# nils-werner/pymf

Measured on AMD Instinct MI355X. Metric: factorize_iters_per_sec, higher is better.
Workload: dtype f32

## Files before the change

pymf_amd/csrc/build.py:

```python
import hashlib
import os
import subprocess
import sys

HERE = os.path.dirname(os.path.abspath(__file__))
OUT = os.path.join(HERE, "libpymf_hip.so")
STAMP = OUT + ".srchash"
DEPS = sorted(f for f in os.listdir(HERE) if f.endswith((".h", ".hip"))) + \
       [os.path.join("..", "..", "include", "pymf_hip.h")]
FLAGS = ["--offload-arch=gfx950", "-O3", "-std=c++17", "-shared", "-fPIC", "-Wno-unused-result",
         "-mllvm", "-amdgpu-mfma-vgpr-form=1"]


def source_hash():
    h = hashlib.sha256()
    h.update(" ".join(FLAGS).encode())
    for d in DEPS:
        p = os.path.join(HERE, d)
        h.update(b"\0" + d.encode() + b"\0")
        with open(p, "rb") as f:
            h.update(f.read())
    return h.hexdigest()


def built_hash():
    try:
        with open(STAMP) as f:
            return f.read().strip()
    except OSError:
        return None


def up_to_date():
    return os.path.exists(OUT) and built_hash() == source_hash()


UNITS = ["pmf_nnls_quad_tu.hip", "pmf_api.hip", "pmf_nnls_tu.hip", "pmf_fused_tu.hip"]


def build(force=False, verbose=True):
    if not force and up_to_date():
        return OUT
    hipcc = os.environ.get("HIPCC", "/opt/rocm/bin/hipcc")
    want = source_hash()
    if os.path.exists(STAMP):
        os.remove(STAMP)
    cflags = [f for f in FLAGS if f != "-shared"]
    objs, procs = [], []
    for u in UNITS:
        obj = os.path.join(HERE, u.replace(".hip", ".o"))
        cmd = [hipcc] + cflags + ["-c", os.path.join(HERE, u), "-o", obj]
        if verbose:
            print(" ".join(cmd), flush=True)
        procs.append((cmd, subprocess.Popen(cmd, cwd=HERE)))
        objs.append(obj)
    for cmd, pr in procs:
        if pr.wait() != 0:
            for _, other in procs:
                if other.poll() is None:
                    other.kill()
            raise subprocess.CalledProcessError(pr.returncode, cmd)
    link = [hipcc, "--offload-arch=gfx950", "-shared", "-fPIC"] + objs + ["-o", OUT, "-lrccl"]
    if verbose:
        print(" ".join(link), flush=True)
    subprocess.check_call(link, cwd=HERE)
    for o in objs:
        os.remove(o)
    if source_hash() != want:
        raise RuntimeError("sources changed while libpymf_hip.so was being built: build again")
    with open(STAMP, "w") as f:
        f.write(want + "\n")
    return OUT


if __name__ == "__main__":
    build(force="--force" in sys.argv)
```

pymf_amd/csrc/pmf_fused.h:

```cpp
#pragma once
#include "pmf_dev.h"
#include <hip/hip_ext.h>
#include "../../include/pymf_hip.h"
#include "pmf_fused_api.h"

#define PMF_GLDS16(gsrc, ldst)                                                            \
  __builtin_amdgcn_global_load_lds((const __attribute__((address_space(1))) void*)(gsrc), \
                                   (__attribute__((address_space(3))) void*)(ldst), 16, 0, 0)

#ifdef PMF_STAMPS
#define PMF_STAMP(var)                                                           \
  do {                                                                           \
    __builtin_amdgcn_sched_barrier(0);                                           \
    asm volatile("s_memtime %0\n\ts_waitcnt lgkmcnt(0)" : "=s"(var)::"memory"); \
    __builtin_amdgcn_sched_barrier(0);                                           \
  } while (0)
#else
#define PMF_STAMP(var) do { } while (0)
#endif


__device__ __forceinline__ void slab_store16(f32x4* p, f32x4 v) { *p = v; }
__device__ __forceinline__ void wrow_store(float* p, float v) { *p = v; }

template <int N>
__device__ __forceinline__ void wait_vmcnt() {
  static_assert(N >= 0 && N < 64, "vmcnt range");
  asm volatile("s_waitcnt vmcnt(%0)" ::"n"(N) : "memory");
}

template <int NT, int NPANEL, int SPLIT = 1>
constexpr size_t fused_smem_bytes() {
  return (size_t)64 * (SPLIT * NPANEL * 16 * NT + 16 * NT + 4 * 16 * NPANEL + 4 * 16) * sizeof(float) +
         (SPLIT == 2 ? (size_t)4 * NT * 1024 : 0);
}

__device__ __forceinline__ int vtile_xor(int row) { return (row ^ ((row & 4) << 1)) & 15; }
__device__ __forceinline__ int vtile_off(int row, int chunk) { return row * 64 + ((chunk ^ vtile_xor(row)) << 2); }
__device__ __forceinline__ f32x4 vtile_read4(const float* base, int row, int chunk) {
  return *reinterpret_cast<const f32x4*>(base + vtile_off(row, chunk));
}

template <int NT, int NPANEL, int MODE, int SPLIT = 1>
__global__ __launch_bounds__(256, 1) void k_nmf_fused(const float* __restrict__ V,
                                                       float* __restrict__ W,
                                                       const float* __restrict__ H,
                                                       const float* __restrict__ G, int blk_per,
                                                       int blk_extra, float lamb,
                                                       float* __restrict__ slab,
                                                       const FusedCtl ctl, int ngp
#ifdef PMF_STAMPS
                                                       , unsigned long long* __restrict__ dbg
#endif
                                                       ) {
  constexpr int KP = 16 * NT;
  static_assert(SPLIT == 1 || (SPLIT == 2 && MODE != FUSED_SNMF), "SPLIT: 1, or 2 for the NMF/BNMF epilogues");
  constexpr int NPT = NPANEL * SPLIT;
  constexpr int NP = 64 * NPT;
  constexpr int NTP = 4 * NPANEL;
  constexpr bool SPREAD = (NPANEL == 4);
  constexpr bool SNMF = (MODE == FUSED_SNMF);
  if (ctl.stop != nullptr && *ctl.stop != 0) return;
#ifdef PMF_STAMPS
  unsigned long long tk0 = 0, tk1 = 0, tk2 = 0, tk3 = 0;
  const unsigned long long rt0 = wall_clock64();
  PMF_STAMP(tk0);
#endif
  extern __shared__ __attribute__((aligned(16))) float smem[];
  float* sH = smem;
  float* sG = sH + NPT * KP * 64;
  float* sVall = sG + KP * 64;
  float* sWall = sVall + 4 * NPANEL * 16 * 64;
  const int tid = threadIdx.x, lane = tid & 63;
  const int wv = __builtin_amdgcn_readfirstlane(tid >> 6);
  const int i = lane & 15, kq = lane >> 4;
  float* sV = sVall + wv * (NPANEL * 1024);
  float* sW = sWall + wv * 1024;
  f32x4* sX = reinterpret_cast<f32x4*>(sWall + 4 * 1024);
  const int half = SPLIT == 2 ? (wv & 1) : 0;
  const int hp = half * NPANEL;

  const int gw = SPLIT == 2 ? blockIdx.x * 2 + (wv >> 1) : blockIdx.x * 4 + wv;
  const int b0 = gw * blk_per + (gw < blk_extra ? gw : blk_extra);
  const int nb = blk_per + (gw < blk_extra ? 1 : 0);
  const int nb_wg = blk_per + (blk_extra > 0 ? 1 : 0);
  constexpr bool interleave = NT == 1;
  const int nw_all = (int)gridDim.x * (SPLIT == 2 ? 2 : 4);
  const int bfirst = interleave ? gw : b0;
  const int bstep = interleave ? nw_all : 1;

  unsigned voff[4], woff[4];
#pragma unroll
  for (int q = 0; q < 4; ++q) {
    const int row = 4 * q + (lane >> 4);
    const int c = (lane & 15) ^ vtile_xor(row);
    voff[q] = (unsigned)(row * NP * 4 + 16 * c);
    woff[q] = (unsigned)(row * KP * 4 + 16 * (4 * c < KP ? c : 0));
  }
  const char* Vb = reinterpret_cast<const char*>(V);
  const char* Wb = reinterpret_cast<const char*>(W);
  auto issue_v = [&](int blk, int p, int q) {
    PMF_GLDS16(Vb + ((size_t)blk * (16 * NP * 4) + (hp + p) * 256) + voff[q], sV + p * 1024 + q * 256);
  };
  auto issue_w = [&](int blk, int q) {
    PMF_GLDS16(Wb + (size_t)blk * (16 * KP * 4) + woff[q], sW + q * 256);
  };

  f32x4 P[NT][NTP];
  f32x4 S[NT][NT];
#pragma unroll
  for (int mt = 0; mt < NT; ++mt) {
#pragma unroll
    for (int nt = 0; nt < NTP; ++nt) P[mt][nt] = f32x4{0.f, 0.f, 0.f, 0.f};
#pragma unroll
    for (int nt = 0; nt < NT; ++nt) S[mt][nt] = f32x4{0.f, 0.f, 0.f, 0.f};
  }

  constexpr int HP = SPLIT * NT;
  constexpr int GP = SNMF ? 0 : NT;
  constexpr int WP = SNMF ? 0 : 4;
  {
    const int drow = lane >> 4, dchunk = lane & 15;
#pragma unroll
    for (int st = 0; st < NPANEL; ++st) {
#pragma unroll
      for (int hh = 0; hh < SPLIT; ++hh)
#pragma unroll
        for (int u = 0; u < NT; ++u) {
          const int p = hh * NPANEL + st, rg = 4 * u + wv;
          const int row = 4 * rg + drow;
          const int bas = NT * (row & 15) + (row >> 4);
          const float* src = H + (size_t)bas * NP + 64 * p + 4 * (dchunk ^ (row & 15));
          PMF_GLDS16(src, sH + p * (KP * 64) + rg * 256);
        }
      if (nb > 0 && (st < NPANEL - 1 || !SPREAD)) {
#pragma unroll
        for (int q = 0; q < 4; ++q) issue_v(bfirst, st, q);
      }
      if (st == 0 && !SNMF && nb > 0) {
#pragma unroll
        for (int q = 0; q < 4; ++q) issue_w(bfirst, q);
      }
    }
#pragma unroll
    for (int u = 0; u < (SNMF ? 0 : NT); ++u) {
      const int rg = 4 * u + wv;
      const int row = 4 * rg + drow;
      const int bas = NT * (row & 15) + (row >> 4);
      int c = dchunk ^ (row & 15);
      if (4 * c >= KP) c = 0;
      if (ngp == 0) {
        PMF_GLDS16(G + bas * KP + 4 * c, sG + rg * 256);
      } else {
        f32x4 g = {0.f, 0.f, 0.f, 0.f};
        for (int w = 0; w < ngp; ++w)
          g += *reinterpret_cast<const f32x4*>(G + (size_t)w * KP * KP + bas * KP + 4 * c);
        *reinterpret_cast<f32x4*>(sG + rg * 256 + drow * 64 + dchunk * 4) = g;
      }
    }
  }
  if (ctl.stop != nullptr && ctl.conv_iter >= 0) {
    double t0 = ctl.tt[0], t1 = ctl.tt[1];
    for (int q = 1; q < ctl.ntt; ++q) { t0 += ctl.tt[2 * q]; t1 += ctl.tt[2 * q + 1]; }
    const double e2 = ctl.vnorm2 - 2.0 * t0 + t1;
    int st = 0;
    if (!(e2 > 1e-3 * ctl.vnorm2)) {
      st = 2;
    } else {
      const double f = sqrt(e2);
      if (blockIdx.x == 0 && tid == 0) ctl.ferr[ctl.conv_iter] = f;
      if (ctl.conv_iter > 1 && fabs(f - ctl.ferr[ctl.conv_iter - 1]) / ctl.nsamp < ctl.eps) st = 1;
    }
    if (st != 0) {
      if (blockIdx.x == 0 && tid == 0) { ctl.stop[1] = ctl.conv_iter; ctl.stop[0] = st; }
      return;
    }
  }
  auto wg_barrier = [&]() {
    asm volatile("s_waitcnt lgkmcnt(0)" ::: "memory");
    __builtin_amdgcn_s_barrier();
    asm volatile("" ::: "memory");
  };
  auto first_stage = [&](int st) {
    if (st >= NPANEL - 1) wait_vmcnt<0>();
    else if (SPREAD) {
      if (st == 0) wait_vmcnt<WP + 2 * (HP + 4) + HP + GP>();
      else if (st == 1) wait_vmcnt<(HP + 4) + HP + GP + 3>();
      else wait_vmcnt<HP + GP + 4>();
    } else {
      if (st == 0) wait_vmcnt<WP + (NPANEL - 1) * (HP + 4) + GP>();
      else if (st == 1) wait_vmcnt<(NPANEL > 2 ? (NPANEL - 2) * (HP + 4) : 0) + GP>();
      else if (st == 2) wait_vmcnt<(NPANEL > 3 ? (NPANEL - 3) * (HP + 4) : 0) + GP>();
      else if (st == 3) wait_vmcnt<(NPANEL > 4 ? (NPANEL - 4) * (HP + 4) : 0) + GP>();
      else wait_vmcnt<0>();
    }
    wg_barrier();
  };
  if (nb == 0) {
    wait_vmcnt<0>();
#pragma unroll
    for (int st = 0; st < NPANEL; ++st) wg_barrier();
  }

  f32x4 fa[2];
  f32x4 fb[2][NT];
  f32x4 bf[2];
  f32x4 wp[NT];
#pragma unroll
  for (int nt = 0; nt < NT; ++nt) wp[nt] = f32x4{0.f, 0.f, 0.f, 0.f};

  constexpr int NSN = 4 * NPANEL;
  constexpr int NSA = SNMF ? NSN : NSN + NT;

#ifdef PMF_STAMPS
  PMF_STAMP(tk1);
  unsigned long long ts0 = 0, ts1 = 0, ts2 = 0, ts3 = 0, ts4 = 0, ts5 = 0;
  unsigned long long acc_wait = 0, acc_a = 0, acc_dma = 0, acc_epi = 0, acc_b = 0;
#endif
  for (int b = 0; b < (SPLIT == 2 ? nb_wg : nb); ++b) {
    if (SPLIT == 2) {
      wg_barrier();
      if (b >= nb) { wg_barrier(); continue; }
    }
    const int blk = bfirst + b * bstep;
    const bool more = (b + 1 < nb);
    PMF_STAMP(ts0);

    f32x4 num[NT], den[NT];
#pragma unroll
    for (int nt = 0; nt < NT; ++nt) {
      num[nt] = f32x4{0.f, 0.f, 0.f, 0.f};
      den[nt] = f32x4{0.f, 0.f, 0.f, 0.f};
    }
    auto load_step = [&](int s, int buf) {
      if (s < NSN) {
        const int p = s >> 2, chunk = 4 * (s & 3) + kq;
        fa[buf] = vtile_read4(sV + p * 1024, i, chunk);
#pragma unroll
        for (int nt = 0; nt < NT; ++nt) fb[buf][nt] = lds_read4(sH + (hp + p) * (KP * 64), 16 * nt + i, chunk);
      } else {
        const int chunk = 4 * (s - NSN) + kq;
        fa[buf] = vtile_read4(sW, i, chunk);
#pragma unroll
        for (int nt = 0; nt < NT; ++nt) fb[buf][nt] = lds_read4(sG, 16 * nt + i, chunk);
      }
    };
    auto wait_panel = [&](int p) {
      if (SPREAD) {
        if (p == 0) wait_vmcnt<8>();
        else if (p == 1) wait_vmcnt<7>();
        else if (p == 2) wait_vmcnt<4>();
        else wait_vmcnt<0>();
      } else {
        if (p == 0) wait_vmcnt<4 * (NPANEL - 1)>();
        else if (p == 1) wait_vmcnt<(NPANEL > 1 ? 4 * (NPANEL - 2) : 0)>();
        else if (p == 2) wait_vmcnt<(NPANEL > 2 ? 4 * (NPANEL - 3) : 0)>();
        else wait_vmcnt<0>();
      }
    };

    const bool first = (b == 0);
    if (first) first_stage(0);
    else wait_panel(0);
    PMF_STAMP(ts1);
    load_step(0, 0);
#pragma unroll
    for (int s = 0; s < NSA; ++s) {
      if (s + 1 < NSA) {
        if (s + 1 < NSN && ((s + 1) & 3) == 0) {
          if (first) first_stage((s + 1) >> 2);
          else wait_panel((s + 1) >> 2);
        }
        load_step(s + 1, (s + 1) & 1);
      }
      const int buf = s & 1;
      if (s < NSN) {
#pragma unroll
        for (int e = 0; e < 4; ++e)
#pragma unroll
          for (int nt = 0; nt < NT; ++nt) num[nt] = mfma16(fa[buf][e], fb[buf][nt][e], num[nt]);
      } else {
#pragma unroll
        for (int e = 0; e < 4; ++e)
#pragma unroll
          for (int nt = 0; nt < NT; ++nt) den[nt] = mfma16(fa[buf][e], fb[buf][nt][e], den[nt]);
      }
      if (SPREAD && s < 4) issue_v(blk, NPANEL - 1, s);
      if (s + 1 < NSA) {
#pragma unroll
        for (int g = 0; g < NT + 1; ++g) {
          __builtin_amdgcn_sched_group_barrier(0x008, NT >= 4 ? 2 : 1, 0);
          __builtin_amdgcn_sched_group_barrier(0x100, 1, 0);
        }
      }
      __builtin_amdgcn_sched_group_barrier(0x008, 4 * NT, 0);
      __builtin_amdgcn_sched_barrier(0);
    }
    if (SPLIT == 2) {
#pragma unroll
      for (int nt = 0; nt < NT; ++nt) sX[(wv * NT + nt) * 64 + lane] = num[nt];
      wg_barrier();
#pragma unroll
      for (int nt = 0; nt < NT; ++nt) num[nt] += sX[((wv ^ 1) * NT + nt) * 64 + lane];
    }
    PMF_STAMP(ts2);
    float wold[NT][4];
    if (!SNMF) {
#pragma unroll
      for (int nt = 0; nt < NT; ++nt)
#pragma unroll
        for (int j = 0; j < 4; ++j) {
          const int row = 4 * kq + j, col = NT * i + nt;
          wold[nt][j] = sW[vtile_off(row, col >> 2) + (col & 3)];
        }
      asm volatile("s_waitcnt lgkmcnt(0)" ::: "memory");
      if (more) {
#pragma unroll
        for (int q = 0; q < 4; ++q) issue_w(blk + bstep, q);
      }
    }
    PMF_STAMP(ts3);

    f32x4 wn[NT];
    float* wdst = W + (size_t)blk * (16 * KP) + (4 * kq) * KP + NT * i;
    if (MODE != FUSED_SNMF) {
      float tnum[NT][4], dd[NT][4], rr[NT][4], qq[NT][4];
      constexpr int NSM = 4 * (NT * (NT + 1) / 2);
      auto s_mfmas = [&](int lo, int hi) {
        if (SPLIT == 1 || half == 0) {
          int q = 0;
#pragma unroll
          for (int j = 0; j < 4; ++j)
#pragma unroll
            for (int nt = 0; nt < NT; ++nt)
#pragma unroll
              for (int mt = 0; mt <= nt; ++mt) {
                if (q >= lo && q < hi) S[mt][nt] = mfma16(wp[mt][j], wp[nt][j], S[mt][nt]);
                ++q;
              }
        }
      };
#pragma unroll
      for (int nt = 0; nt < NT; ++nt)
#pragma unroll
        for (int j = 0; j < 4; ++j) {
          const float w0 = wold[nt][j];
          if (MODE == FUSED_BNMF) {
            tnum[nt][j] = num[nt][j] + (3.0f * lamb) * (w0 * w0);
            dd[nt][j] = ((den[nt][j] + (2.0f * lamb) * (w0 * w0 * w0)) + lamb * w0) + PMF_EPS_DEN;
          } else if (MODE == FUSED_RNMF) {
            const float x = num[nt][j];
            tnum[nt][j] = fabsf(x) - x;
            dd[nt][j] = 2.0f * den[nt][j];
          } else {
            tnum[nt][j] = w0 * num[nt][j];
            dd[nt][j] = den[nt][j] + PMF_EPS_DEN;
          }
        }
      s_mfmas(0, NSM / 5);
      __builtin_amdgcn_sched_barrier(0);
#pragma unroll
      for (int nt = 0; nt < NT; ++nt)
#pragma unroll
        for (int j = 0; j < 4; ++j) rr[nt][j] = __builtin_amdgcn_rcpf(dd[nt][j]);
      s_mfmas(NSM / 5, 2 * NSM / 5);
      __builtin_amdgcn_sched_barrier(0);
#pragma unroll
      for (int nt = 0; nt < NT; ++nt)
#pragma unroll
        for (int j = 0; j < 4; ++j) qq[nt][j] = tnum[nt][j] * rr[nt][j];
      s_mfmas(2 * NSM / 5, 3 * NSM / 5);
      __builtin_amdgcn_sched_barrier(0);
#pragma unroll
      for (int nt = 0; nt < NT; ++nt)
#pragma unroll
        for (int j = 0; j < 4; ++j) tnum[nt][j] = fmaf(-dd[nt][j], qq[nt][j], tnum[nt][j]);
      s_mfmas(3 * NSM / 5, 4 * NSM / 5);
      __builtin_amdgcn_sched_barrier(0);
#pragma unroll
      for (int nt = 0; nt < NT; ++nt)
#pragma unroll
        for (int j = 0; j < 4; ++j) {
          float w = fmaf(tnum[nt][j], rr[nt][j], qq[nt][j]);
          if (MODE == FUSED_BNMF) w = wold[nt][j] * w;
          if (MODE == FUSED_RNMF) w = dd[nt][j] != 0.f ? wold[nt][j] * w : 0.f;
          wn[nt][j] = w;
          if (SPLIT == 1 || half == 0) wrow_store(&wdst[j * KP + nt], w);
        }
      s_mfmas(4 * NSM / 5, NSM);
      __builtin_amdgcn_sched_barrier(0);
    } else {
#pragma unroll
      for (int nt = 0; nt < NT; ++nt)
#pragma unroll
        for (int j = 0; j < 4; ++j) {
          const float w = num[nt][j];
          wn[nt][j] = w;
          wrow_store(&wdst[j * KP + nt], w);
#pragma unroll
          for (int mt = 0; mt <= nt; ++mt) S[mt][nt] = mfma16(wp[mt][j], wp[nt][j], S[mt][nt]);
        }
    }
#pragma unroll
    for (int nt = 0; nt < NT; ++nt) wp[nt] = wn[nt];

    PMF_STAMP(ts4);
    auto load_bf = [&](int s, int buf) {
      const int p = s >> 2, row = 4 * kq + (s & 3);
      bf[buf] = vtile_read4(sV + p * 1024, row, i);
    };
    load_bf(0, 0);
#pragma unroll
    for (int s = 0; s < NSN; ++s) {
      if (s + 1 < NSN) load_bf(s + 1, (s + 1) & 1);
      const int p = s >> 2, j = s & 3, buf = s & 1;
#pragma unroll
      for (int mt = 0; mt < NT; ++mt)
#pragma unroll
        for (int nt = 0; nt < 4; ++nt)
          P[mt][4 * p + nt] = mfma16(wn[mt][j], bf[buf][nt], P[mt][4 * p + nt]);
      if (SPREAD) {
        if (p >= 1 && more) issue_v(blk + bstep, p - 1, j);
      }
      if (s + 1 < NSN) {
        __builtin_amdgcn_sched_group_barrier(0x008, NT >= 2 ? 2 : 1, 0);
        __builtin_amdgcn_sched_group_barrier(0x100, 1, 0);
      }
      __builtin_amdgcn_sched_barrier(0);
      if (!SPREAD && j == 3) {
        asm volatile("s_waitcnt lgkmcnt(0)" ::: "memory");
        if (more) {
#pragma unroll
          for (int q = 0; q < 4; ++q) issue_v(blk + bstep, p, q);
        }
      }
    }
    if (SPREAD) asm volatile("s_waitcnt lgkmcnt(0)" ::: "memory");
#ifdef PMF_STAMPS
    PMF_STAMP(ts5);
    acc_wait += ts1 - ts0; acc_a += ts2 - ts1; acc_dma += ts3 - ts2; acc_epi += ts4 - ts3; acc_b += ts5 - ts4;
#endif
  }
#ifdef PMF_STAMPS
  PMF_STAMP(tk2);
#endif
  if (SPLIT == 1 || half == 0) {
#pragma unroll
    for (int j = 0; j < 4; ++j)
#pragma unroll
      for (int nt = 0; nt < NT; ++nt)
#pragma unroll
        for (int mt = 0; mt <= nt; ++mt) S[mt][nt] = mfma16(wp[mt][j], wp[nt][j], S[mt][nt]);
  }

  constexpr int NTU = NT * NTP + NT * (NT + 1) / 2;
  __syncthreads();
  f32x4* ex = reinterpret_cast<f32x4*>(smem);
  static_assert((size_t)2 * NTU * 64 * 16 <= fused_smem_bytes<NT, NPANEL, SPLIT>(), "exchange fits");
  auto put = [&](int region) {
    f32x4* dst = ex + (size_t)region * NTU * 64 + lane;
#pragma unroll
    for (int mt = 0; mt < NT; ++mt) {
#pragma unroll
      for (int nt = 0; nt < NTP; ++nt) dst[(mt * NTP + nt) * 64] = P[mt][nt];
#pragma unroll
      for (int nt = mt; nt < NT; ++nt)
        dst[(NT * NTP + mt * NT - (mt * (mt - 1)) / 2 + (nt - mt)) * 64] = S[mt][nt];
    }
  };
  auto add = [&](int region) {
    const f32x4* src = ex + (size_t)region * NTU * 64 + lane;
#pragma unroll
    for (int mt = 0; mt < NT; ++mt) {
#pragma unroll
      for (int nt = 0; nt < NTP; ++nt) P[mt][nt] += src[(mt * NTP + nt) * 64];
#pragma unroll
      for (int nt = mt; nt < NT; ++nt)
        S[mt][nt] += src[(NT * NTP + mt * NT - (mt * (mt - 1)) / 2 + (nt - mt)) * 64];
    }
  };
  if (wv >= 2) put(wv - 2);
  __syncthreads();
  if (wv < 2) add(wv);
  __syncthreads();
  if (wv < 2) put(wv);
  __syncthreads();
  if (SPLIT == 1) {
    f32x4* out = reinterpret_cast<f32x4*>(slab) + (size_t)blockIdx.x * NTU * 64 + lane;
    for (int t = wv; t < NTU; t += 4)
      slab_store16(&out[t * 64], ex[t * 64 + lane] + ex[(size_t)NTU * 64 + t * 64 + lane]);
  } else {
    constexpr int NTPT = 4 * NPT, NTUT = NT * NTPT + NT * (NT + 1) / 2;
    f32x4* out = reinterpret_cast<f32x4*>(slab) + (size_t)blockIdx.x * NTUT * 64 + lane;
    for (int t = wv; t < 2 * NT * NTP; t += 4) {
      const int h = t / (NT * NTP), q = t % (NT * NTP), mt = q / NTP, nt = q % NTP;
      slab_store16(&out[(mt * NTPT + h * NTP + nt) * 64], ex[(size_t)h * NTU * 64 + q * 64 + lane]);
    }
    for (int t = wv; t < NT * (NT + 1) / 2; t += 4)
      slab_store16(&out[(NT * NTPT + t) * 64], ex[(NT * NTP + t) * 64 + lane]);
  }
#ifdef PMF_STAMPS
  PMF_STAMP(tk3);
  if (dbg && lane == 0) {
    unsigned long long* d = dbg + ((size_t)blockIdx.x * 4 + wv) * 12;
    d[0] = acc_wait; d[1] = acc_a; d[2] = acc_dma; d[3] = acc_epi; d[4] = acc_b; d[5] = (unsigned long long)nb;
    d[6] = tk1 - tk0; d[7] = tk3 - tk2;
    d[8] = rt0; d[9] = wall_clock64(); d[10] = tk3 - tk0; d[11] = tk2 - tk1;
  }
#endif
}

#ifndef PMF_FUSED_KERNEL_ONLY
static inline bool fused_shape_ok(int NT, int np) {
  const int npanel = np / 64;
  if (np % 64 != 0 || npanel < 1) return false;
  const int max_panels = NT == 1 ? 6 : NT == 2 ? 5 : NT == 4 ? 4 : 0;
  return npanel <= max_panels;
}

static inline bool fused_shape_split(int NT, int np) {
  if (NT == 2) return np == 384 || np == 512;
  if (NT == 1) return np == 512;
  return false;
}

static inline int fused_grid_for(int NT, int np, int64_t mp, bool allow_split = true) {
  const bool split = allow_split && !fused_shape_ok(NT, np) && fused_shape_split(NT, np);
  if (!fused_shape_ok(NT, np) && !split) return 0;
  int dev = 0, cus = 256;
  hipDeviceProp_t prop;
  if (hipGetDevice(&dev) == hipSuccess && hipGetDeviceProperties(&prop, dev) == hipSuccess)
    cus = prop.multiProcessorCount;
  const int64_t nblk = mp / 16;
  int64_t wgs = split ? (nblk + 1) / 2 : (nblk + 3) / 4;
  if (wgs > cus) wgs = cus;
  return (int)wgs;
}

static inline const char* fused_kernel_name(int NT, int np, int mode = FUSED_NMF) {
  static char buf[64];
  const bool split = !fused_shape_ok(NT, np) && fused_shape_split(NT, np) && mode != FUSED_SNMF;
  snprintf(buf, sizeof(buf), "k_nmf_fused<%d,%d%s%s>", NT, split ? np / 128 : np / 64,
           mode == FUSED_SNMF ? ",snmf" : mode == FUSED_BNMF ? ",bnmf" : mode == FUSED_RNMF ? ",rnmf" : "", split ? ",SPLIT 2" : "");
  return buf;
}

template <int NT, int NPANEL, int MODE, int SPLIT = 1>
static int launch_fused_t(hipStream_t s, const float* V, float* W, const float* H, const float* G,
                          int64_t mp, int wgs, float lamb, float* slab, const FusedCtl& ctl, int ngp,
                          hipEvent_t e0, hipEvent_t e1) {
  const int nblk = (int)(mp / 16), nw = wgs * (SPLIT == 2 ? 2 : 4);
  const int blk_per = nblk / nw, blk_extra = nblk % nw;
  const size_t smem = fused_smem_bytes<NT, NPANEL, SPLIT>();
  static bool attr_done_dev[PMF_MAX_DEVICES] = {};
  bool& attr_done = attr_done_dev[pmf_current_device()];
  if (!attr_done) {
    if (hipFuncSetAttribute(reinterpret_cast<const void*>(&k_nmf_fused<NT, NPANEL, MODE, SPLIT>),
                            hipFuncAttributeMaxDynamicSharedMemorySize, (int)smem) != hipSuccess)
      return PMF_EHIP;
    attr_done = true;
  }
  if (e0 != nullptr && e1 != nullptr)
    hipExtLaunchKernelGGL((k_nmf_fused<NT, NPANEL, MODE, SPLIT>), dim3(wgs), dim3(256), (uint32_t)smem, s, e0, e1, 0u, V, W, H, G, blk_per,
                          blk_extra, lamb, slab, ctl, ngp);
  else
    hipLaunchKernelGGL((k_nmf_fused<NT, NPANEL, MODE, SPLIT>), dim3(wgs), dim3(256), smem, s, V, W, H, G, blk_per,
                       blk_extra, lamb, slab, ctl, ngp);
  return PMF_OK;
}

static inline int launch_fused(hipStream_t s, int mode, int NT, int np, const float* V, float* W,
                               const float* H, const float* G, int64_t mp, int wgs, float lamb,
                               float* slab, const FusedCtl& ctl, int ngp = 0, hipEvent_t e0 = nullptr, hipEvent_t e1 = nullptr) {
  if (!fused_shape_ok(NT, np) && fused_shape_split(NT, np) && mode != FUSED_SNMF) {
    const int skey = NT * 10 + np / 128;
#define PMF_FUSED_SPLIT_CASE(K, A, B)                                                                   \
  case K:                                                                                               \
    return mode == FUSED_BNMF   ? launch_fused_t<A, B, FUSED_BNMF, 2>(s, V, W, H, G, mp, wgs, lamb, slab, ctl, ngp, e0, e1) \
           : mode == FUSED_RNMF ? launch_fused_t<A, B, FUSED_RNMF, 2>(s, V, W, H, G, mp, wgs, lamb, slab, ctl, ngp, e0, e1) \
                                : launch_fused_t<A, B, FUSED_NMF, 2>(s, V, W, H, G, mp, wgs, lamb, slab, ctl, ngp, e0, e1);
    switch (skey) {
      PMF_FUSED_SPLIT_CASE(14, 1, 4)
      PMF_FUSED_SPLIT_CASE(23, 2, 3)
      PMF_FUSED_SPLIT_CASE(24, 2, 4)
    }
#undef PMF_FUSED_SPLIT_CASE
    return PMF_EINVAL;
  }
  const int key = NT * 10 + np / 64;
#define PMF_FUSED_CASE(K, A, B)                                                                  \
  case K:                                                                                        \
    return mode == FUSED_SNMF   ? launch_fused_t<A, B, FUSED_SNMF>(s, V, W, H, G, mp, wgs, lamb, slab, ctl, ngp, e0, e1) \
           : mode == FUSED_BNMF ? launch_fused_t<A, B, FUSED_BNMF>(s, V, W, H, G, mp, wgs, lamb, slab, ctl, ngp, e0, e1) \
           : mode == FUSED_RNMF ? launch_fused_t<A, B, FUSED_RNMF>(s, V, W, H, G, mp, wgs, lamb, slab, ctl, ngp, e0, e1) \
                                : launch_fused_t<A, B, FUSED_NMF>(s, V, W, H, G, mp, wgs, lamb, slab, ctl, ngp, e0, e1);
  switch (key) {
    PMF_FUSED_CASE(11, 1, 1)
    PMF_FUSED_CASE(12, 1, 2)
    PMF_FUSED_CASE(13, 1, 3)
    PMF_FUSED_CASE(14, 1, 4)
    PMF_FUSED_CASE(15, 1, 5)
    PMF_FUSED_CASE(16, 1, 6)
    PMF_FUSED_CASE(21, 2, 1)
    PMF_FUSED_CASE(22, 2, 2)
    PMF_FUSED_CASE(23, 2, 3)
    PMF_FUSED_CASE(24, 2, 4)
    PMF_FUSED_CASE(25, 2, 5)
    PMF_FUSED_CASE(41, 4, 1)
    PMF_FUSED_CASE(42, 4, 2)
    PMF_FUSED_CASE(43, 4, 3)
    PMF_FUSED_CASE(44, 4, 4)
  }
#undef PMF_FUSED_CASE
  return PMF_EINVAL;
}
#endif
```

Before: 1611.

## Peel first block and software-pipeline next-block loads across fused NMF loop

Turns the block loop body into a lambda and peels the first iteration with a compile-time flag. The next block's W prefetch, its first V panel wait and its first LDS fragment load now sit inside the tail of the previous block. The old-W reads move into the last A-stage step, and the first B-stage fragment load is interleaved with the epilogue stages. Prefetches always issue, reloading the current block when there is no next one, so the `more` branch goes away, and a final vmcnt wait is added before the exchange. Asm hints keep the base address scalar and the lane offset in vector registers, and SLP vectorization is disabled for this unit. This adds redundant DMA traffic on the last block and makes the ordering assumptions fragile.

Measured after the change: 1620 (median of 6 runs). Within noise of the previous version (+0.5%).

```diff
diff --git a/pymf_amd/csrc/build.py b/pymf_amd/csrc/build.py
--- a/pymf_amd/csrc/build.py
+++ b/pymf_amd/csrc/build.py
@@ -12,9 +12,17 @@
          "-mllvm", "-amdgpu-mfma-vgpr-form=1"]
 
 
+UNIT_FLAGS = {"pmf_fused_tu.hip": ["-fno-slp-vectorize"]}
+
+
+def unit_flags(unit):
+    return [f for f in FLAGS if f != "-shared"] + UNIT_FLAGS.get(unit, [])
+
+
 def source_hash():
     h = hashlib.sha256()
     h.update(" ".join(FLAGS).encode())
+    h.update(repr(sorted(UNIT_FLAGS.items())).encode())
     for d in DEPS:
         p = os.path.join(HERE, d)
         h.update(b"\0" + d.encode() + b"\0")
@@ -45,11 +53,10 @@
     want = source_hash()
     if os.path.exists(STAMP):
         os.remove(STAMP)
-    cflags = [f for f in FLAGS if f != "-shared"]
     objs, procs = [], []
     for u in UNITS:
         obj = os.path.join(HERE, u.replace(".hip", ".o"))
-        cmd = [hipcc] + cflags + ["-c", os.path.join(HERE, u), "-o", obj]
+        cmd = [hipcc] + unit_flags(u) + ["-c", os.path.join(HERE, u), "-o", obj]
         if verbose:
             print(" ".join(cmd), flush=True)
         procs.append((cmd, subprocess.Popen(cmd, cwd=HERE)))
diff --git a/pymf_amd/csrc/pmf_fused.h b/pymf_amd/csrc/pmf_fused.h
--- a/pymf_amd/csrc/pmf_fused.h
+++ b/pymf_amd/csrc/pmf_fused.h
@@ -1,6 +1,7 @@
 #pragma once
 #include "pmf_dev.h"
 #include <hip/hip_ext.h>
+#include <type_traits>
 #include "../../include/pymf_hip.h"
 #include "pmf_fused_api.h"
 
@@ -99,11 +100,20 @@
   }
   const char* Vb = reinterpret_cast<const char*>(V);
   const char* Wb = reinterpret_cast<const char*>(W);
+  auto lane_off = [&](unsigned off, int blk) {
+    asm("" : "+v"(off) : "s"(blk));
+    return off;
+  };
+  auto row_base = [&](const char* p) {
+    unsigned long long a = reinterpret_cast<unsigned long long>(p);
+    asm("" : "+s"(a));
+    return reinterpret_cast<const char*>(a);
+  };
   auto issue_v = [&](int blk, int p, int q) {
-    PMF_GLDS16(Vb + ((size_t)blk * (16 * NP * 4) + (hp + p) * 256) + voff[q], sV + p * 1024 + q * 256);
+    PMF_GLDS16(row_base(Vb + ((size_t)blk * (16 * NP * 4) + (hp + p) * 256)) + lane_off(voff[q], blk), sV + p * 1024 + q * 256);
   };
   auto issue_w = [&](int blk, int q) {
-    PMF_GLDS16(Wb + (size_t)blk * (16 * KP * 4) + woff[q], sW + q * 256);
+    PMF_GLDS16(row_base(Wb + (size_t)blk * (16 * KP * 4)) + lane_off(woff[q], blk), sW + q * 256);
   };
 
   f32x4 P[NT][NTP];
@@ -217,13 +227,14 @@
   unsigned long long ts0 = 0, ts1 = 0, ts2 = 0, ts3 = 0, ts4 = 0, ts5 = 0;
   unsigned long long acc_wait = 0, acc_a = 0, acc_dma = 0, acc_epi = 0, acc_b = 0;
 #endif
-  for (int b = 0; b < (SPLIT == 2 ? nb_wg : nb); ++b) {
+  auto block = [&](int b, auto first_tag) __attribute__((always_inline)) {
+    constexpr bool first = decltype(first_tag)::value;
     if (SPLIT == 2) {
       wg_barrier();
-      if (b >= nb) { wg_barrier(); continue; }
+      if (b >= nb) { wg_barrier(); return; }
     }
     const int blk = bfirst + b * bstep;
-    const bool more = (b + 1 < nb);
+    const int nxt = (b + 1 < nb) ? blk + bstep : blk;
     PMF_STAMP(ts0);
 
     f32x4 num[NT], den[NT];
@@ -259,11 +270,12 @@
       }
     };
 
-    const bool first = (b == 0);
-    if (first) first_stage(0);
-    else wait_panel(0);
+    if (first) {
+      first_stage(0);
+      load_step(0, 0);
+    }
     PMF_STAMP(ts1);
-    load_step(0, 0);
+    float wold[NT][4];
 #pragma unroll
     for (int s = 0; s < NSA; ++s) {
       if (s + 1 < NSA) {
@@ -286,6 +298,20 @@
           for (int nt = 0; nt < NT; ++nt) den[nt] = mfma16(fa[buf][e], fb[buf][nt][e], den[nt]);
       }
       if (SPREAD && s < 4) issue_v(blk, NPANEL - 1, s);
+      if (!SNMF && s == NSA - 1) {
+#pragma unroll
+        for (int j = 0; j < 4; ++j)
+#pragma unroll
+          for (int nt = 0; nt < NT; ++nt) {
+            const int row = 4 * kq + j, col = NT * i + nt;
+            wold[nt][j] = sW[vtile_off(row, col >> 2) + (col & 3)];
+          }
+#pragma unroll
+        for (int j = 0; j < 4; ++j) {
+          __builtin_amdgcn_sched_group_barrier(0x008, NT >= 4 ? 2 : 1, 0);
+          __builtin_amdgcn_sched_group_barrier(0x100, 1, 0);
+        }
+      }
       if (s + 1 < NSA) {
 #pragma unroll
         for (int g = 0; g < NT + 1; ++g) {
@@ -304,23 +330,12 @@
       for (int nt = 0; nt < NT; ++nt) num[nt] += sX[((wv ^ 1) * NT + nt) * 64 + lane];
     }
     PMF_STAMP(ts2);
-    float wold[NT][4];
-    if (!SNMF) {
-#pragma unroll
-      for (int nt = 0; nt < NT; ++nt)
-#pragma unroll
-        for (int j = 0; j < 4; ++j) {
-          const int row = 4 * kq + j, col = NT * i + nt;
-          wold[nt][j] = sW[vtile_off(row, col >> 2) + (col & 3)];
-        }
-      asm volatile("s_waitcnt lgkmcnt(0)" ::: "memory");
-      if (more) {
-#pragma unroll
-        for (int q = 0; q < 4; ++q) issue_w(blk + bstep, q);
-      }
-    }
     PMF_STAMP(ts3);
 
+    auto load_bf = [&](int s, int buf) {
+      const int p = s >> 2, row = 4 * kq + (s & 3);
+      bf[buf] = vtile_read4(sV + p * 1024, row, i);
+    };
     f32x4 wn[NT];
     float* wdst = W + (size_t)blk * (16 * KP) + (4 * kq) * KP + NT * i;
     if (MODE != FUSED_SNMF) {
@@ -340,55 +355,80 @@
               }
         }
       };
-#pragma unroll
-      for (int nt = 0; nt < NT; ++nt)
-#pragma unroll
-        for (int j = 0; j < 4; ++j) {
-          const float w0 = wold[nt][j];
-          if (MODE == FUSED_BNMF) {
-            tnum[nt][j] = num[nt][j] + (3.0f * lamb) * (w0 * w0);
-            dd[nt][j] = ((den[nt][j] + (2.0f * lamb) * (w0 * w0 * w0)) + lamb * w0) + PMF_EPS_DEN;
-          } else if (MODE == FUSED_RNMF) {
-            const float x = num[nt][j];
-            tnum[nt][j] = fabsf(x) - x;
-            dd[nt][j] = 2.0f * den[nt][j];
-          } else {
-            tnum[nt][j] = w0 * num[nt][j];
-            dd[nt][j] = den[nt][j] + PMF_EPS_DEN;
+      auto stage0 = [&]() {
+#pragma unroll
+        for (int nt = 0; nt < NT; ++nt)
+#pragma unroll
+          for (int j = 0; j < 4; ++j) {
+            const float w0 = wold[nt][j];
+            if (MODE == FUSED_BNMF) {
+              tnum[nt][j] = num[nt][j] + (3.0f * lamb) * (w0 * w0);
+              dd[nt][j] = ((den[nt][j] + (2.0f * lamb) * (w0 * w0 * w0)) + lamb * w0) + PMF_EPS_DEN;
+            } else if (MODE == FUSED_RNMF) {
+              const float x = num[nt][j];
+              tnum[nt][j] = fabsf(x) - x;
+              dd[nt][j] = 2.0f * den[nt][j];
+            } else {
+              tnum[nt][j] = w0 * num[nt][j];
+              dd[nt][j] = den[nt][j] + PMF_EPS_DEN;
+            }
           }
-        }
-      s_mfmas(0, NSM / 5);
-      __builtin_amdgcn_sched_barrier(0);
-#pragma unroll
-      for (int nt = 0; nt < NT; ++nt)
-#pragma unroll
-        for (int j = 0; j < 4; ++j) rr[nt][j] = __builtin_amdgcn_rcpf(dd[nt][j]);
-      s_mfmas(NSM / 5, 2 * NSM / 5);
-      __builtin_amdgcn_sched_barrier(0);
-#pragma unroll
-      for (int nt = 0; nt < NT; ++nt)
-#pragma unroll
-        for (int j = 0; j < 4; ++j) qq[nt][j] = tnum[nt][j] * rr[nt][j];
-      s_mfmas(2 * NSM / 5, 3 * NSM / 5);
-      __builtin_amdgcn_sched_barrier(0);
-#pragma unroll
-      for (int nt = 0; nt < NT; ++nt)
-#pragma unroll
-        for (int j = 0; j < 4; ++j) tnum[nt][j] = fmaf(-dd[nt][j], qq[nt][j], tnum[nt][j]);
-      s_mfmas(3 * NSM / 5, 4 * NSM / 5);
-      __builtin_amdgcn_sched_barrier(0);
-#pragma unroll
-      for (int nt = 0; nt < NT; ++nt)
-#pragma unroll
-        for (int j = 0; j < 4; ++j) {
-          float w = fmaf(tnum[nt][j], rr[nt][j], qq[nt][j]);
-          if (MODE == FUSED_BNMF) w = wold[nt][j] * w;
-          if (MODE == FUSED_RNMF) w = dd[nt][j] != 0.f ? wold[nt][j] * w : 0.f;
-          wn[nt][j] = w;
-          if (SPLIT == 1 || half == 0) wrow_store(&wdst[j * KP + nt], w);
-        }
-      s_mfmas(4 * NSM / 5, NSM);
-      __builtin_amdgcn_sched_barrier(0);
+      };
+      auto prefetch_w = [&]() {
+        asm volatile("s_waitcnt lgkmcnt(0)" ::: "memory");
+#pragma unroll
+        for (int q = 0; q < 4; ++q) issue_w(nxt, q);
+      };
+      auto stage1 = [&]() {
+#pragma unroll
+        for (int nt = 0; nt < NT; ++nt)
+#pragma unroll
+          for (int j = 0; j < 4; ++j) rr[nt][j] = __builtin_amdgcn_rcpf(dd[nt][j]);
+      };
+      auto stage2 = [&]() {
+#pragma unroll
+        for (int nt = 0; nt < NT; ++nt)
+#pragma unroll
+          for (int j = 0; j < 4; ++j) qq[nt][j] = tnum[nt][j] * rr[nt][j];
+      };
+      auto stage3 = [&]() {
+#pragma unroll
+        for (int nt = 0; nt < NT; ++nt)
+#pragma unroll
+          for (int j = 0; j < 4; ++j) tnum[nt][j] = fmaf(-dd[nt][j], qq[nt][j], tnum[nt][j]);
+      };
+      auto stage4 = [&]() {
+#pragma unroll
+        for (int j = 0; j < 4; ++j)
+#pragma unroll
+          for (int nt = 0; nt < NT; ++nt) {
+            float w = fmaf(tnum[nt][j], rr[nt][j], qq[nt][j]);
+            if (MODE == FUSED_BNMF) w = wold[nt][j] * w;
+            if (MODE == FUSED_RNMF) w = dd[nt][j] != 0.f ? wold[nt][j] * w : 0.f;
+            wn[nt][j] = w;
+            if (SPLIT == 1 || half == 0) wrow_store(&wdst[j * KP + nt], w);
+          }
+      };
+      {
+        stage0();
+        s_mfmas(0, NSM / 5);
+        __builtin_amdgcn_sched_barrier(0);
+        prefetch_w();
+        stage1();
+        s_mfmas(NSM / 5, 2 * NSM / 5);
+        __builtin_amdgcn_sched_barrier(0);
+        stage2();
+        s_mfmas(2 * NSM / 5, 3 * NSM / 5);
+        __builtin_amdgcn_sched_barrier(0);
+        stage3();
+        s_mfmas(3 * NSM / 5, 4 * NSM / 5);
+        __builtin_amdgcn_sched_barrier(0);
+        if (MODE == FUSED_NMF) load_bf(0, 0);
+        stage4();
+        s_mfmas(4 * NSM / 5, NSM);
+        __builtin_amdgcn_sched_barrier(0);
+        if (MODE != FUSED_NMF) load_bf(0, 0);
+      }
     } else {
 #pragma unroll
       for (int nt = 0; nt < NT; ++nt)
@@ -405,11 +445,7 @@
     for (int nt = 0; nt < NT; ++nt) wp[nt] = wn[nt];
 
     PMF_STAMP(ts4);
-    auto load_bf = [&](int s, int buf) {
-      const int p = s >> 2, row = 4 * kq + (s & 3);
-      bf[buf] = vtile_read4(sV + p * 1024, row, i);
-    };
-    load_bf(0, 0);
+    if (MODE == FUSED_SNMF) load_bf(0, 0);
 #pragma unroll
     for (int s = 0; s < NSN; ++s) {
       if (s + 1 < NSN) load_bf(s + 1, (s + 1) & 1);
@@ -420,18 +456,29 @@
         for (int nt = 0; nt < 4; ++nt)
           P[mt][4 * p + nt] = mfma16(wn[mt][j], bf[buf][nt], P[mt][4 * p + nt]);
       if (SPREAD) {
-        if (p >= 1 && more) issue_v(blk + bstep, p - 1, j);
+        if (p >= 1) issue_v(nxt, p - 1, j);
       }
       if (s + 1 < NSN) {
         __builtin_amdgcn_sched_group_barrier(0x008, NT >= 2 ? 2 : 1, 0);
         __builtin_amdgcn_sched_group_barrier(0x100, 1, 0);
+      } else if (SPREAD) {
+        wait_panel(0);
+        load_step(0, 0);
+        __builtin_amdgcn_sched_group_barrier(0x010, 1, 0);
+#pragma unroll
+        for (int g = 0; g < NT + 1; ++g) {
+          __builtin_amdgcn_sched_group_barrier(0x008, NT >= 4 ? 2 : 1, 0);
+          __builtin_amdgcn_sched_group_barrier(0x100, 1, 0);
+        }
       }
       __builtin_amdgcn_sched_barrier(0);
       if (!SPREAD && j == 3) {
         asm volatile("s_waitcnt lgkmcnt(0)" ::: "memory");
-        if (more) {
-#pragma unroll
-          for (int q = 0; q < 4; ++q) issue_v(blk + bstep, p, q);
+#pragma unroll
+        for (int q = 0; q < 4; ++q) issue_v(nxt, p, q);
+        if (s + 1 == NSN) {
+          wait_panel(0);
+          load_step(0, 0);
         }
       }
     }
@@ -440,7 +487,10 @@
     PMF_STAMP(ts5);
     acc_wait += ts1 - ts0; acc_a += ts2 - ts1; acc_dma += ts3 - ts2; acc_epi += ts4 - ts3; acc_b += ts5 - ts4;
 #endif
-  }
+  };
+  const int nloop = SPLIT == 2 ? nb_wg : nb;
+  if (nloop > 0) block(0, std::true_type{});
+  for (int b = 1; b < nloop; ++b) block(b, std::false_type{});
 #ifdef PMF_STAMPS
   PMF_STAMP(tk2);
 #endif
@@ -454,6 +504,7 @@
   }
 
   constexpr int NTU = NT * NTP + NT * (NT + 1) / 2;
+  wait_vmcnt<0>();
   __syncthreads();
   f32x4* ex = reinterpret_cast<f32x4*>(smem);
   static_assert((size_t)2 * NTU * 64 * 16 <= fused_smem_bytes<NT, NPANEL, SPLIT>(), "exchange fits");
```
